# NTT123/vietTTS

Hardware: NVIDIA H100
Metric: audio_samples_per_sec (higher is better)
Workload: dtype f32 (bf16x3 split products on wgmma tensor cores, fp32 accumulate/storage)

## Files before the change

### viettts_b200/csrc/tc_conv.cu

```cuda
#include <cuda_bf16.h>

#include <algorithm>

#include "tc_common.cuh"
#include "vtts_internal.cuh"

namespace {

using namespace tcx;

constexpr int NCWG = 2;
constexpr int NCONS = NCWG * 128;
constexpr int PROD_WARP = NCONS / 32;
constexpr int NCONV = 96;
constexpr int NTHREADS = NCONS + 32 + NCONV;
constexpr int NA = 4;
constexpr int HALO = 64;
constexpr int PAIR_OVERLAP = 16;
constexpr int NQ = 2;
constexpr int NREADERS = (NCONS + NCONV) / 32;

constexpr int SUB_CG = 4;
constexpr int SUB_HALO = 1;
constexpr int SUB_RS = NCWG * 64 + SUB_HALO;
constexpr int SUB_CSB = SUB_RS * 64 + 32;
constexpr int SUB_STAGE = SUB_CG * SUB_CSB;
static_assert(SUB_RS * 4 % 32 == 4 && SUB_CSB / 4 % 32 == 24, "bank-conflict-free converter stores");

template <int N, int MW, int PAIRF, bool STAGED = false, bool SUB = false>
struct TcCfg {
  static constexpr int R = 64 * MW * NCWG;
  static constexpr int R_OUT = R - PAIR_OVERLAP;
  static constexpr int RA = R + HALO;
  static constexpr int A_STAGE = RA * 64;
  static constexpr int NAS = SUB ? (N == 64 ? 4 : 2) : NA;
  static constexpr int A_BYTES = SUB ? NAS * SUB_STAGE : NA * A_STAGE;
  static constexpr int W_STAGE = N * 64;
  static constexpr int NW = N == 256 ? 4 : 8;
  static constexpr int NCH2 = PAIRF ? N / 16 : 0;
  static constexpr int EPI_NC = N < 128 ? N : 128;
  static constexpr int EPI_LD = EPI_NC + 8;
  static constexpr int EPI_WG = 64 * EPI_LD + N;
  static constexpr int EPI_STAGE = STAGED ? NCWG * EPI_WG * 4 : 0;
  static constexpr int SMEM_BYTES =
      A_BYTES + NW * W_STAGE + NCH2 * A_STAGE + EPI_STAGE + (2 * NA + 2 * NW + 2 * NQ) * 8 + NQ * 4 + 1024;
  static_assert(SMEM_BYTES <= 227 * 1024, "shared memory of one CTA");
};

struct Ring {
  uint32_t s = 0, p = 0;
  template <int NS>
  __device__ __forceinline__ void next() { if (++s == NS) { s = 0; p ^= 1; } }
};

struct Tile {
  int pi, b, tt;
};
__device__ __forceinline__ Tile decode_tile(int t, int nprob, int tiles_per_row) {
  Tile d;
  d.pi = t % nprob; t /= nprob;
  d.tt = t % tiles_per_row;
  d.b = t / tiles_per_row;
  return d;
}

__device__ __forceinline__ int take_ticket(int* sched, int ntiles) {
  const int t = (int)gridDim.x + atomicAdd(&sched[0], 1);
  if (t < ntiles) return t;
  __threadfence();
  if (atomicAdd(&sched[1], 1) == (int)gridDim.x - 1) {
    atomicExch(&sched[0], 0);
    atomicExch(&sched[1], 0);
  }
  return -1;
}

struct TileQueue {
  int* id;
  uint64_t* full;
  uint64_t* empty;
  Ring r;
  __device__ __forceinline__ void put(int t, int* err, long long& acc) {
    mbar_wait_t(&empty[r.s], r.p ^ 1, err, 6, acc);
    id[r.s] = t;
    mbar_arrive(&full[r.s]);
    r.next<NQ>();
  }
  __device__ __forceinline__ int get(int* err, long long& acc) {
    int t = 0;
    if ((threadIdx.x & 31) == 0) {
      mbar_wait_t(&full[r.s], r.p, err, 6, acc);
      t = id[r.s];
      mbar_arrive(&empty[r.s]);
    }
    r.next<NQ>();
    return __shfl_sync(0xffffffffu, t, 0);
  }
};

__device__ __forceinline__ float div3_rn(float s) {
  constexpr float y = 0x1.555556p-2f;
  const float q0 = __fmul_rn(s, y);
  const float q1 = __fmaf_rn(__fmaf_rn(-q0, 3.0f, s), y, q0);
  return (s == 0.f || fabsf(s) == __int_as_float(0x7f800000)) ? s : q1;
}

template <int QN, int RS, int CSB, bool F16, bool LOADS_FIRST = false>
__device__ __forceinline__ void convert_rows(uint8_t* stage, int ct, const float* x0, const float* x1, const float* x2, int ld, int ch0,
                                             int row_base, int rows, int lo, int valid, int pre_mode, float slope) {
  static_assert(NCONV % QN == 0, "whole rows per converter step");
  constexpr int RSTEP = NCONV / QN, RA = RS;
  const int q = ct % QN;
  const int r0 = ct / QN;
  uint8_t* st = stage + (q >> 2) * CSB + (((q >> 1) & 1) * RA) * 16 + (q & 1) * 8;
  const int coff = ch0 + q * 4;
  constexpr int U = 8;
  for (int rr0 = r0; rr0 < rows; rr0 += RSTEP * U) {
    float4 v[U];
    if constexpr (LOADS_FIRST) {
      float4 a[U], bb[U];
      bool in[U];
#pragma unroll
      for (int u = 0; u < U; ++u) {
        const int rr = rr0 + u * RSTEP;
        const int t = row_base + rr;
        in[u] = rr < rows && t >= lo && t < valid;
        v[u] = a[u] = bb[u] = make_float4(0.f, 0.f, 0.f, 0.f);
        if (in[u]) {
          const size_t off = (size_t)t * ld + coff;
          v[u] = ldg_pf256(x0 + off);
          if (pre_mode == 2) {
            a[u] = ldg_pf256(x1 + off);
            bb[u] = ldg_pf256(x2 + off);
          }
        }
      }
#pragma unroll
      for (int u = 0; u < U; ++u) {
        if (in[u] && pre_mode == 2) {
          v[u].x = div3_rn((v[u].x + a[u].x) + bb[u].x);
          v[u].y = div3_rn((v[u].y + a[u].y) + bb[u].y);
          v[u].z = div3_rn((v[u].z + a[u].z) + bb[u].z);
          v[u].w = div3_rn((v[u].w + a[u].w) + bb[u].w);
        }
      }
    } else {
#pragma unroll
      for (int u = 0; u < U; ++u) {
        const int rr = rr0 + u * RSTEP;
        const int t = row_base + rr;
        v[u] = make_float4(0.f, 0.f, 0.f, 0.f);
        if (rr < rows && t >= lo && t < valid) {
          const size_t off = (size_t)t * ld + coff;
          v[u] = ldg_pf256(x0 + off);
          if (pre_mode == 2) {
            const float4 a = ldg_pf256(x1 + off);
            const float4 bb = ldg_pf256(x2 + off);
            v[u].x = ((v[u].x + a.x) + bb.x) / 3.0f;
            v[u].y = ((v[u].y + a.y) + bb.y) / 3.0f;
            v[u].z = ((v[u].z + a.z) + bb.z) / 3.0f;
            v[u].w = ((v[u].w + a.w) + bb.w) / 3.0f;
          }
        }
      }
    }
#pragma unroll
    for (int u = 0; u < U; ++u) {
      const int rr = rr0 + u * RSTEP;
      if (rr < rows) {
        float4 x = v[u];
        if (pre_mode >= 1) {
          x.x = lrelu(x.x, slope); x.y = lrelu(x.y, slope); x.z = lrelu(x.z, slope); x.w = lrelu(x.w, slope);
        }
        if constexpr (F16) {
          *reinterpret_cast<uint2*>(st + (size_t)rr * 16) = f16x4_sat(x);
        } else {
          uint2 hi, lo;
          split4(x, hi, lo);
          *reinterpret_cast<uint2*>(st + (size_t)rr * 16) = hi;
          *reinterpret_cast<uint2*>(st + (size_t)(2 * RA + rr) * 16) = lo;
        }
      }
    }
  }
}

template <int RA, bool F16>
__device__ __forceinline__ void convert_chunk(uint8_t* stage, int ct, const float* x0, const float* x1, const float* x2, int ld, int c,
                                              int row_base, int rows, int lo, int valid, int pre_mode, float slope) {
  convert_rows<4, RA, 0, F16>(stage, ct, x0, x1, x2, ld, c * 16, row_base, rows, lo, valid, pre_mode, slope);
}

template <int N, int NW, bool F16>
__device__ __forceinline__ void produce_weights(uint8_t* w_st, uint64_t* w_full, uint64_t* w_empty, Ring& rw, const void* wpk, int nch,
                                                int k, int* err, long long& wait_acc) {
  constexpr int WB = F16 ? N * 32 : N * 64;
  const uint8_t* src = reinterpret_cast<const uint8_t*>(wpk);
  for (int i = 0; i < nch * k; ++i) {
    mbar_wait_t(&w_empty[rw.s], rw.p ^ 1, err, 4, wait_acc);
    mbar_expect_tx(&w_full[rw.s], WB);
    bulk_g2s(w_st + rw.s * (N * 64), src + (size_t)i * WB, WB, &w_full[rw.s]);
    rw.next<NW>();
  }
}

template <int N, int MW, int RA, int NW, bool A_FROM_RING, bool A_REGS, bool F16>
__device__ __forceinline__ void consume(float (&acc)[MW][N / 2], int wg, uint32_t a_st_u32, uint64_t* a_full, uint64_t* a_empty, Ring& ra,
                                        uint32_t w_st_u32, uint64_t* w_full, uint64_t* w_empty, Ring& rw, int nch, int k, int dil,
                                        int* err, long long& w_a, long long& w_w) {
  const uint64_t a_tmpl = make_desc(0, RA * 16, 128);
  const uint64_t b_tmpl = make_desc(0, (F16 ? 1 : 2) * N * 16, 128);
  const bool lane0 = (threadIdx.x & 31) == 0;
  int pend_w = -1, pend_a = -1;
  for (int c = 0; c < nch; ++c) {
    uint32_t a_base;
    if constexpr (A_FROM_RING) {
      mbar_wait_t(&a_full[ra.s], ra.p, err, 2, w_a);
      a_base = a_st_u32 + ra.s * (RA * 64);
    } else {
      a_base = a_st_u32 + c * (RA * 64);
    }
    for (int j = 0; j < k; ++j) {
      mbar_wait_t(&w_full[rw.s], rw.p, err, 3, w_w);
      const uint32_t w_base = w_st_u32 + rw.s * (N * 64);
      const uint64_t b_hi = b_tmpl | (uint64_t)(w_base >> 4);
      const uint64_t b_lo = b_tmpl | (uint64_t)((w_base + N * 16) >> 4);
      const uint32_t first = (c | j) != 0 ? 1u : 0u;
      if constexpr (A_REGS) {
        static_assert(!A_FROM_RING && !F16, "register A operand: bf16 planes of the fixed buffer");
        const int lane = threadIdx.x & 31, wl = (threadIdx.x >> 5) & 3;
        uint32_t fa_hi[MW][4], fa_lo[MW][4];
#pragma unroll
        for (int mt = 0; mt < MW; ++mt) {
          const int row = (wg * MW + mt) * 64 + wl * 16 + ((lane >> 3) & 1) * 8 + (lane & 7) + j * dil;
          const uint32_t addr = a_base + ((lane >> 4) * RA + row) * 16;
          ldmatrix_x4(fa_hi[mt], addr);
          ldmatrix_x4(fa_lo[mt], addr + 2 * RA * 16);
        }
        wgmma_fence();
#pragma unroll
        for (int mt = 0; mt < MW; ++mt) {
          wgmma_rs<N>(acc[mt], fa_hi[mt], b_hi, first);
          wgmma_rs<N>(acc[mt], fa_hi[mt], b_lo, 1u);
          wgmma_rs<N>(acc[mt], fa_lo[mt], b_hi, 1u);
        }
        wgmma_commit();
        wgmma_wait<0>();
        if (lane == 0) mbar_arrive(&w_empty[rw.s]);
        rw.next<NW>();
        continue;
      }
      wgmma_fence();
#pragma unroll
      for (int mt = 0; mt < MW; ++mt) {
        const uint32_t row = a_base + ((wg * MW + mt) * 64 + j * dil) * 16;
        const uint64_t a_hi = a_tmpl | (uint64_t)(row >> 4);
        const uint64_t a_lo = a_tmpl | (uint64_t)((row + 2 * RA * 16) >> 4);
        if constexpr (F16) {
          wgmma<N, true>(acc[mt], a_hi, b_hi, first);
        } else {
          wgmma<N>(acc[mt], a_hi, b_hi, first);
          wgmma<N>(acc[mt], a_hi, b_lo, 1u);
          wgmma<N>(acc[mt], a_lo, b_hi, 1u);
        }
      }
      wgmma_commit();
      wgmma_wait<1>();
      if (lane0) {
        if (pend_w >= 0) mbar_arrive(&w_empty[pend_w]);
        if (pend_a >= 0) mbar_arrive(&a_empty[pend_a]);
      }
      pend_w = (int)rw.s;
      pend_a = (A_FROM_RING && j == k - 1) ? (int)ra.s : -1;
      rw.next<NW>();
    }
    if constexpr (A_FROM_RING) ra.next<NA>();
  }
  wgmma_wait<0>();
  if (lane0) {
    if (pend_w >= 0) mbar_arrive(&w_empty[pend_w]);
    if (pend_a >= 0) mbar_arrive(&a_empty[pend_a]);
  }
}

template <int N, int NW, int NAS, bool F16>
__device__ __forceinline__ void consume_rows(float (&acc)[N / 2], int wg, uint32_t a_st_u32, uint64_t* a_full, uint64_t* a_empty, Ring& ra,
                                             uint32_t w_st_u32, uint64_t* w_full, uint64_t* w_empty, Ring& rw, int nch, int k, int dil,
                                             int* err, long long& w_a, long long& w_w) {
  const uint64_t a_tmpl = make_desc(0, SUB_RS * 16, 128);
  const uint64_t b_tmpl = make_desc(0, (F16 ? 1 : 2) * N * 16, 128);
  const bool lane0 = (threadIdx.x & 31) == 0;
  int pend_w = -1, pend_a = -1;
  for (int c0 = 0; c0 < nch; c0 += SUB_CG) {
    mbar_wait_t(&a_full[ra.s], ra.p, err, 2, w_a);
    const uint32_t a_blk = a_st_u32 + ra.s * SUB_STAGE + wg * 64 * 16;
    for (int cl = 0; cl < SUB_CG; ++cl) {
      for (int j = 0; j < k; ++j) {
        mbar_wait_t(&w_full[rw.s], rw.p, err, 3, w_w);
        const uint32_t w_base = w_st_u32 + rw.s * (N * 64);
        const uint64_t b_hi = b_tmpl | (uint64_t)(w_base >> 4);
        const uint64_t b_lo = b_tmpl | (uint64_t)((w_base + N * 16) >> 4);
        const uint32_t first = ((c0 + cl) | j) != 0 ? 1u : 0u;
        const uint32_t row = a_blk + cl * SUB_CSB + j * dil * 16;
        const uint64_t a_hi = a_tmpl | (uint64_t)(row >> 4);
        const uint64_t a_lo = a_tmpl | (uint64_t)((row + 2 * SUB_RS * 16) >> 4);
        wgmma_fence();
        if constexpr (F16) {
          wgmma<N, true>(acc, a_hi, b_hi, first);
        } else {
          wgmma<N>(acc, a_hi, b_hi, first);
          wgmma<N>(acc, a_hi, b_lo, 1u);
          wgmma<N>(acc, a_lo, b_hi, 1u);
        }
        wgmma_commit();
        wgmma_wait<1>();
        if (lane0) {
          if (pend_w >= 0) mbar_arrive(&w_empty[pend_w]);
          if (pend_a >= 0) mbar_arrive(&a_empty[pend_a]);
        }
        pend_w = (int)rw.s;
        pend_a = (cl == SUB_CG - 1 && j == k - 1) ? (int)ra.s : -1;
        rw.next<NW>();
      }
    }
    ra.next<NAS>();
  }
  wgmma_wait<0>();
  if (lane0) {
    if (pend_w >= 0) mbar_arrive(&w_empty[pend_w]);
    if (pend_a >= 0) mbar_arrive(&a_empty[pend_a]);
  }
}

__device__ __forceinline__ void cp_async16(void* smem_dst, const void* gsrc) {
  asm volatile("cp.async.cg.shared.global [%0], [%1], 16;" ::"r"(smem_u32(smem_dst)), "l"(gsrc) : "memory");
}
__device__ __forceinline__ void cp_async_commit() { asm volatile("cp.async.commit_group;" ::: "memory"); }
__device__ __forceinline__ void cp_async_wait_all() { asm volatile("cp.async.wait_all;" ::: "memory"); }

__device__ __forceinline__ void init_barriers(uint64_t* bars, int nw) {
  uint64_t* a_full = bars;
  uint64_t* a_empty = bars + NA;
  uint64_t* w_full = bars + 2 * NA;
  uint64_t* w_empty = bars + 2 * NA + nw;
  uint64_t* q_full = bars + 2 * NA + 2 * nw;
  uint64_t* q_empty = q_full + NQ;
  for (int i = 0; i < NA; ++i) { mbar_init(&a_full[i], NCONV); mbar_init(&a_empty[i], NCONS / 32); }
  for (int i = 0; i < nw; ++i) { mbar_init(&w_full[i], 1); mbar_init(&w_empty[i], NCONS / 32); }
  for (int i = 0; i < NQ; ++i) { mbar_init(&q_full[i], 1); mbar_init(&q_empty[i], NREADERS); }
  asm volatile("fence.mbarrier_init.release.cluster;" ::: "memory");
}

__device__ __forceinline__ TileQueue tile_queue(uint64_t* bars, int nw) {
  uint64_t* q_full = bars + 2 * NA + 2 * nw;
  return TileQueue{reinterpret_cast<int*>(q_full + 2 * NQ), q_full, q_full + NQ, Ring{}};
}

// ... 157 lines not shown
      }
      const long long t_epi0 = clock64();
      if constexpr (EPI == 0) {
        wait_pass();
#pragma unroll
        for (int mt = 0; mt < MW; ++mt) {
          const int blk = blk_row(mt);
          if (SUB ? sub_elem(L, P, blk, 0) >= e_lim : !row_ok(blk)) break;
#pragma unroll
          for (int nh = 0; nh < N / EPI_NC; ++nh) {
            if (mt + nh > 0 && P.resid) {
              fetch_pass(mt, nh);
              wait_pass();
            }
#pragma unroll
            for (int jn = 0; jn < EPI_NC / 8; ++jn) {
              const int col = jn * 8 + fc, e = (nh * (EPI_NC / 8) + jn) * 4;
              const float2 bi = *reinterpret_cast<const float2*>(stg_bias + nh * EPI_NC + col);
#pragma unroll
              for (int h = 0; h < 2; ++h) {
                float2* s = reinterpret_cast<float2*>(stg + (fr + 8 * h) * EPI_LD + col);
                float2 o = make_float2(acc[mt][e + 2 * h] + bi.x, acc[mt][e + 2 * h + 1] + bi.y);
                if (P.resid) {
                  const float2 r = *s;
                  o.x += r.x; o.y += r.y;
                }
                *s = o;
              }
            }
            named_bar(2 + wg, 128);
#pragma unroll
            for (int i = 0; i < NQ4; ++i) {
              const int row = i * RPS + dr, tau = blk + row;
              const int e = (tau * ostride + ooff) * L.out_ld + oe0 + nh * EPI_NC + dq * 4;
              if (elem_ok(tau, e))
                *reinterpret_cast<float4*>(P.out + out_base + e) = *reinterpret_cast<const float4*>(stg + row * EPI_LD + dq * 4);
            }
            named_bar(2 + wg, 128);
          }
        }
      } else {
        const int row_w = tau0 + wg * MW * 64 + (warp & 3) * 16 + (lane >> 2);
#pragma unroll
        for (int mt = 0; mt < MW; ++mt)
#pragma unroll
          for (int h = 0; h < 2; ++h) {
            const int tau = row_w + mt * 64 + 8 * h;
            if (!row_ok(tau)) continue;
            const size_t orow = out_base + (size_t)(tau * ostride + ooff) * L.out_ld;
#pragma unroll
            for (int jn = 0; jn < N / 8; ++jn) {
              const int col = jn * 8 + 2 * (lane & 3);
              if (col >= n_valid) continue;
              float2 o = make_float2(acc[mt][jn * 4 + 2 * h], acc[mt][jn * 4 + 2 * h + 1]);
              const float2 bi = __ldg(reinterpret_cast<const float2*>(P.bias + col));
              o.x += bi.x; o.y += bi.y;
              if (P.bn_mean) {
                const float2 mu = __ldg(reinterpret_cast<const float2*>(P.bn_mean + col));
                const float2 iv = __ldg(reinterpret_cast<const float2*>(P.bn_inv + col));
                const float2 of = __ldg(reinterpret_cast<const float2*>(P.bn_off + col));
                o.x = (o.x - mu.x) * iv.x + of.x; o.y = (o.y - mu.y) * iv.y + of.y;
              }
              if (post_act == 1) { o.x = tanhf(o.x); o.y = tanhf(o.y); }
              else if (post_act == 2) { o.x = fmaxf(o.x, 0.f); o.y = fmaxf(o.y, 0.f); }
              if (P.resid) {
                const float2 r = __ldg(reinterpret_cast<const float2*>(P.resid + orow + col));
                o.x += r.x; o.y += r.y;
              }
              *reinterpret_cast<float2*>(P.out + orow + col) = o;
            }
          }
      }
      t_epi += clock64() - t_epi0;
    TILE_LOOP_END
    if (L.dbg && tid == 0) {
      long long* d = L.dbg + (size_t)blockIdx.x * 16;
      d[0] = clock64() - t_begin; d[1] = t_epi; d[2] = w_a; d[3] = w_w;
    }
  }
#undef TILE_LOOP_BEGIN
#undef TILE_LOOP_END
}

template <int N, int MW, bool A2_REGS, bool F16>
__global__ void __launch_bounds__(NTHREADS, 1) tc_pair_kernel(const __grid_constant__ TcPairLaunch L) {
  using Cfg = TcCfg<N, MW, 1>;
  constexpr int R = Cfg::R, R_OUT = Cfg::R_OUT, RA = Cfg::RA, NW = Cfg::NW, NCH = N / 16;
  extern __shared__ uint8_t smem_raw[];
  uint8_t* smem = (uint8_t*)(((uintptr_t)smem_raw + 1023) & ~(uintptr_t)1023);
  uint8_t* a_st = smem;
  uint8_t* w_st = smem + NA * Cfg::A_STAGE;
  uint8_t* mid = w_st + NW * Cfg::W_STAGE;
  uint64_t* bars = reinterpret_cast<uint64_t*>(mid + Cfg::NCH2 * Cfg::A_STAGE);
  uint64_t* a_full = bars;
  uint64_t* a_empty = bars + NA;
  uint64_t* w_full = bars + 2 * NA;
  uint64_t* w_empty = bars + 2 * NA + NW;

  const int tid = threadIdx.x;
  const int warp = __shfl_sync(0xffffffffu, tid >> 5, 0);
  if (tid == 0) init_barriers(bars, NW);
  __syncthreads();

#define TILE_LOOP_BEGIN                                                   \
  for (int tile; (tile = next_tile()) >= 0;) {                            \
    const Tile td = decode_tile(tile, L.nprob, L.tiles_per_row);        \
    const int b = td.b;                                                    \
    const int tau0 = td.tt * R_OUT;                                        \
    int valid = L.T_rows;                                                 \
    if (L.len) {                                                          \
      const int v = L.len[b] * L.len_mul;                                 \
      valid = v < valid ? v : valid;                                      \
    }                                                                     \
    if (tau0 >= valid) continue;                                          \
    const TcPairProb& P = L.p[td.pi];                                      \
    const int k = P.k, dil = P.dil, h2 = (k - 1) / 2;
#define TILE_LOOP_END }

  if (warp == PROD_WARP) {
    if ((tid & 31) == 0) {
      Ring rw;
      long long w_e = 0;
      PRODUCER_TILES
      TILE_LOOP_BEGIN
        (void)b; (void)tau0; (void)dil; (void)h2;
        produce_weights<N, NW, F16>(w_st, w_full, w_empty, rw, P.w1pk, NCH, k, L.err, w_e);
        produce_weights<N, NW, F16>(w_st, w_full, w_empty, rw, P.w2pk, NCH, k, L.err, w_e);
      TILE_LOOP_END
    }
  } else if (warp > PROD_WARP) {
    const int ct = tid - NCONS - 32;
    Ring ra;
    long long w_ae = 0;
    READER_TILES
    TILE_LOOP_BEGIN
      const float* x = P.x + (size_t)b * L.T_rows * N;
      const int row_base = tau0 - h2 - (k - 1) * dil / 2;
      for (int c = 0; c < NCH; ++c) {
        mbar_wait_t(&a_empty[ra.s], ra.p ^ 1, L.err, 5, w_ae);
        convert_chunk<RA, F16>(a_st + ra.s * Cfg::A_STAGE, ct, x, nullptr, nullptr, N, c, row_base, R + (k - 1) * dil, 0, valid, 1, L.slope);
        fence_proxy_async();
        mbar_arrive(&a_full[ra.s]);
        ra.next<NA>();
      }
    TILE_LOOP_END
  } else {
    const int wg = warp >> 2, lane = tid & 31;
    float acc[MW][N / 2];
    Ring ra, rw;
    long long w_a = 0, w_w = 0;
    const long long t_begin = clock64();
    const float slope = L.slope;
    READER_TILES
    TILE_LOOP_BEGIN
      consume<N, MW, RA, NW, true, false, F16>(acc, wg, smem_u32(a_st), a_full, a_empty, ra, smem_u32(w_st), w_full, w_empty, rw, NCH, k, dil,
                                               L.err, w_a, w_w);
      const int lr_w = wg * MW * 64 + (warp & 3) * 16 + (lane >> 2);
#pragma unroll
      for (int mt = 0; mt < MW; ++mt)
#pragma unroll
        for (int h = 0; h < 2; ++h) {
          const int lr = lr_w + mt * 64 + 8 * h;
          const int u = tau0 - h2 + lr;
          const bool inside = u >= 0 && u < valid;
#pragma unroll
          for (int jn = 0; jn < N / 8; ++jn) {
            const int col = jn * 8 + 2 * (lane & 3);
            const float2 bi = __ldg(reinterpret_cast<const float2*>(P.b1 + col));
            const float v0 = inside ? lrelu(acc[mt][jn * 4 + 2 * h] + bi.x, slope) : 0.f;
            const float v1 = inside ? lrelu(acc[mt][jn * 4 + 2 * h + 1] + bi.y, slope) : 0.f;
            uint8_t* dst = mid + (col >> 4) * Cfg::A_STAGE + (((col >> 3) & 1) * RA + lr) * 16 + (col & 7) * 2;
            if constexpr (F16) {
              *reinterpret_cast<uint32_t*>(dst) = f16x2_sat(v0, v1);
            } else {
              const __nv_bfloat162 hi = __floats2bfloat162_rn(v0, v1);
              const __nv_bfloat162 lo = __floats2bfloat162_rn(v0 - __low2float(hi), v1 - __high2float(hi));
              *reinterpret_cast<__nv_bfloat162*>(dst) = hi;
              *reinterpret_cast<__nv_bfloat162*>(dst + 2 * RA * 16) = lo;
            }
          }
        }
      fence_proxy_async();
      named_bar(1, NCONS);
      consume<N, MW, RA, NW, false, A2_REGS, F16>(acc, wg, smem_u32(mid), a_full, a_empty, ra, smem_u32(w_st), w_full, w_empty, rw, NCH, k, 1,
                                                  L.err, w_a, w_w);
      named_bar(1, NCONS);
      const float* x = P.x + (size_t)b * L.T_rows * N;
      float* out = P.out + (size_t)b * L.T_rows * N;
#pragma unroll
      for (int mt = 0; mt < MW; ++mt)
#pragma unroll
        for (int h = 0; h < 2; ++h) {
          const int lr = lr_w + mt * 64 + 8 * h;
          const int tau = tau0 + lr;
          if (lr >= R_OUT || tau >= valid) continue;
#pragma unroll
          for (int jn = 0; jn < N / 8; ++jn) {
            const int col = jn * 8 + 2 * (lane & 3);
            const float2 bi = __ldg(reinterpret_cast<const float2*>(P.b2 + col));
            const float2 r = __ldg(reinterpret_cast<const float2*>(x + (size_t)tau * N + col));
            float2 o;
            o.x = acc[mt][jn * 4 + 2 * h] + bi.x + r.x;
            o.y = acc[mt][jn * 4 + 2 * h + 1] + bi.y + r.y;
            *reinterpret_cast<float2*>(out + (size_t)tau * N + col) = o;
          }
        }
    TILE_LOOP_END
    if (L.dbg && tid == 0) {
      long long* d = L.dbg + (size_t)blockIdx.x * 16;
      d[0] = clock64() - t_begin; d[2] = w_a; d[3] = w_w;
    }
  }
#undef TILE_LOOP_BEGIN
#undef TILE_LOOP_END
}

template <bool F16>
__global__ void pack_w_kernel(const float* __restrict__ w, uint16_t* __restrict__ dst, int k, int Cin, int Cout_total, int n0, int N) {
  const size_t total = (size_t)k * Cin * N;
  for (size_t idx = blockIdx.x * (size_t)blockDim.x + threadIdx.x; idx < total; idx += (size_t)gridDim.x * blockDim.x) {
    const int n = idx % N;
    const int i = (idx / N) % Cin;
    const int j = idx / ((size_t)N * Cin);
    const float v = (n0 + n) < Cout_total ? w[((size_t)j * Cin + i) * Cout_total + n0 + n] : 0.f;
    const int c = i / 16, kh = (i % 16) / 8, e = i % 8;
    if constexpr (F16) {
      const size_t blk = ((size_t)c * k + j) * (size_t)(2 * N * 8);
      dst[blk + ((size_t)kh * N + n) * 8 + e] = (uint16_t)(f16x2_sat(v, 0.f) & 0xffffu);
      continue;
    }
    const __nv_bfloat16 hi = __float2bfloat16_rn(v);
    const __nv_bfloat16 lo = __float2bfloat16_rn(v - __bfloat162float(hi));
    const size_t blk = ((size_t)c * k + j) * (size_t)(4 * N * 8);
    dst[blk + ((size_t)(kh * 2 + 0) * N + n) * 8 + e] = __bfloat16_as_ushort(hi);
    dst[blk + ((size_t)(kh * 2 + 1) * N + n) * 8 + e] = __bfloat16_as_ushort(lo);
  }
}

template <int N, int EPI, int MW, bool F16, bool SUB = false>
int launch_cfg(vtts_ctx* ctx, TcLaunch& L, cudaStream_t st) {
  using Cfg = TcCfg<N, MW, 0, EPI == 0, SUB>;
  static bool attr_done_dev[64] = {};
  if (!attr_done_dev[ctx->device & 63]) {
    VTTS_CUDA(cudaFuncSetAttribute(tc_conv_kernel<N, EPI, MW, F16, SUB>, cudaFuncAttributeMaxDynamicSharedMemorySize, Cfg::SMEM_BYTES));
    attr_done_dev[ctx->device & 63] = true;
  }
  for (int i = 0; i < L.nprob; ++i)
    if ((L.p[i].k - 1) * L.p[i].dil > (SUB ? SUB_HALO : HALO)) return ctx->fail(VTTS_ERR_BAD_ARG, "tc_conv: halo too large");
  if (SUB && L.Cin % (SUB_CG * 16)) return ctx->fail(VTTS_ERR_BAD_ARG, "tc_conv: sub-row output needs Cin %% %d == 0, not %d", SUB_CG * 16, L.Cin);
  std::stable_sort(L.p, L.p + L.nprob, [](const TcProb& a, const TcProb& b) { return a.k > b.k; });
  L.tiles_per_row = ((L.tile_rows > 0 ? L.tile_rows : L.T_rows) + Cfg::R - 1) / Cfg::R;
  L.ntiles = L.nprob * L.tiles_per_row * L.B;
  const int grid = L.ntiles < ctx->sm_count ? L.ntiles : ctx->sm_count;
  tc_conv_kernel<N, EPI, MW, F16, SUB><<<grid, NTHREADS, Cfg::SMEM_BYTES, st>>>(L);
  ctx->launches++;
  VTTS_CUDA(cudaGetLastError());
  return VTTS_OK;
}

template <int N>
int launch_n(vtts_ctx* ctx, TcLaunch& L, cudaStream_t st) {
  constexpr int MW = N >= 256 ? 1 : (N == 128 ? 2 : 4);
  bool generic = L.post_act != 0 || (L.n_valid > 0 && L.n_valid < N);
  bool rb = false;
  for (int i = 0; i < L.nprob; ++i) {
    generic |= L.p[i].bn_mean != nullptr;
    rb |= L.p[i].rb != nullptr;
  }
  if ((rb || L.out_sub) && generic) return ctx->fail(VTTS_ERR_BAD_ARG, "tc_conv: per-row bounds and sub-row output use the plain epilogue");
  if (L.out_sub < 0 || (L.out_sub && (L.out_sub % 4 || L.out_ld % L.out_sub)))
    return ctx->fail(VTTS_ERR_BAD_ARG, "tc_conv: output rows of %d floats in tile rows of %d", L.out_sub, L.out_ld);
  if (!generic) {
    const int row_w = L.out_sub ? L.out_sub : L.out_ld;
    if ((int64_t)L.rows_out * row_w > INT32_MAX) return ctx->fail(VTTS_ERR_BAD_ARG, "tc_conv: %d output rows of %d", L.rows_out, row_w);
    bool aligned = L.out_ld % 4 == 0;
    for (int i = 0; i < L.nprob; ++i) aligned &= (((uintptr_t)L.p[i].out | (uintptr_t)L.p[i].resid | (uintptr_t)L.p[i].bias) & 15) == 0;
    if (!aligned) return ctx->fail(VTTS_ERR_BAD_ARG, "tc_conv: the plain epilogue needs 16-byte aligned out / resid rows and bias (out_ld %d)", L.out_ld);
  }
  if (L.f16 && generic) return ctx->fail(VTTS_ERR_BAD_ARG, "tc_conv: fp16 operands use the plain epilogue");
  if (L.f16) return L.out_sub ? launch_cfg<N, 0, MW, true, true>(ctx, L, st) : launch_cfg<N, 0, MW, true>(ctx, L, st);
  if (generic) return launch_cfg<N, 1, MW, false>(ctx, L, st);
  return L.out_sub ? launch_cfg<N, 0, MW, false, true>(ctx, L, st) : launch_cfg<N, 0, MW, false>(ctx, L, st);
}

template <int N, int MW, bool A2_REGS, bool F16 = false>
int launch_pair(vtts_ctx* ctx, TcPairLaunch& L, cudaStream_t st) {
  using Cfg = TcCfg<N, MW, 1>;
  static bool attr_done_dev[64] = {};
  if (!attr_done_dev[ctx->device & 63]) {
    VTTS_CUDA(cudaFuncSetAttribute(tc_pair_kernel<N, MW, A2_REGS, F16>, cudaFuncAttributeMaxDynamicSharedMemorySize, Cfg::SMEM_BYTES));
    attr_done_dev[ctx->device & 63] = true;
  }
  for (int i = 0; i < L.nprob; ++i)
    if (L.p[i].k - 1 > PAIR_OVERLAP || (L.p[i].k - 1) * L.p[i].dil > HALO) return ctx->fail(VTTS_ERR_BAD_ARG, "tc_pair: halo too large");
  std::stable_sort(L.p, L.p + L.nprob, [](const TcPairProb& a, const TcPairProb& b) { return a.k > b.k; });
  L.tiles_per_row = (L.T_rows + Cfg::R_OUT - 1) / Cfg::R_OUT;
  L.ntiles = L.nprob * L.tiles_per_row * L.B;
  const int grid = L.ntiles < ctx->sm_count ? L.ntiles : ctx->sm_count;
  tc_pair_kernel<N, MW, A2_REGS, F16><<<grid, NTHREADS, Cfg::SMEM_BYTES, st>>>(L);
  ctx->launches++;
  VTTS_CUDA(cudaGetLastError());
  return VTTS_OK;
}

}

size_t vtts_tc_packed_elems(int k, int Cin, int N, bool f16) { return (size_t)k * Cin * N * (f16 ? 1 : 2); }

int vtts_tc_pack_weights(vtts_ctx* ctx, const float* w, void* dst, int k, int Cin, int Cout_total, int n0, int N, bool f16) {
  if (f16) pack_w_kernel<true><<<256, 256>>>(w, reinterpret_cast<uint16_t*>(dst), k, Cin, Cout_total, n0, N);
  else pack_w_kernel<false><<<256, 256>>>(w, reinterpret_cast<uint16_t*>(dst), k, Cin, Cout_total, n0, N);
  VTTS_CUDA(cudaGetLastError());
  return VTTS_OK;
}

int vtts_tc_tile_n(int Cout) { return Cout <= 32 ? 32 : (Cout <= 64 ? 64 : (Cout <= 128 ? 128 : 256)); }

size_t vtts_tc_conv_packed_bytes(int k, int Cin, int Cout, bool f16) {
  const int N = vtts_tc_tile_n(Cout), nt = (Cout + N - 1) / N;
  return ((vtts_tc_packed_elems(k, Cin, N, f16) * 2 + 255) & ~size_t(255)) * nt;
}

int vtts_tc_pack_conv(vtts_ctx* ctx, const float* w, int k, int Cin, int Cout, bool f16, char*& cursor, std::vector<void*>& out) {
  const int N = vtts_tc_tile_n(Cout), nt = (Cout + N - 1) / N;
  for (int t = 0; t < nt; ++t) {
    int rc = vtts_tc_pack_weights(ctx, w, cursor, k, Cin, Cout, t * N, N, f16);
    if (rc) return rc;
    out.push_back(cursor);
    cursor += (vtts_tc_packed_elems(k, Cin, N, f16) * 2 + 255) & ~size_t(255);
  }
  return VTTS_OK;
}

int vtts_conv_dispatch(vtts_ctx* ctx, const ConvLaunch& L, void* const* wpk, cudaStream_t st) {
  if (ctx->precision == VTTS_PRECISION_FP32 || wpk == nullptr) return vtts_launch_conv(ctx, L, st);
  const int N = vtts_tc_tile_n(L.Cout), nt = (L.Cout + N - 1) / N;
  TcLaunch TL;
  auto reset = [&]() {
    memset(&TL, 0, sizeof(TL));
    TL.Cin = L.Cin; TL.N = N; TL.in_ld = L.Cin; TL.out_ld = L.Cout; TL.B = L.B; TL.T_rows = L.T_rows; TL.rows_out = L.rows_out;
    TL.len = L.len; TL.len_mul = L.len_mul; TL.pre_mode = L.pre_mode; TL.pre_slope = L.pre_slope; TL.post_act = L.post_act;
    TL.n_valid = (L.Cout % N) ? (L.Cout % N) : N;
  };
  reset();
  for (int pass = 0; pass < 2; ++pass) {
    const bool partial = pass == 1;
    if (partial && (L.Cout % N) == 0) break;
    reset();
    TL.n_valid = partial ? (L.Cout % N) : N;
    for (int pi = 0; pi < L.nprob; ++pi) {
      const ConvProb& cp = L.p[pi];
      for (int t = 0; t < nt; ++t) {
        const bool is_partial = (t == nt - 1) && (L.Cout % N) != 0;
        if (is_partial != partial) continue;
        const int n0 = t * N;
        TcProb q;
        memset(&q, 0, sizeof(q));
        q.x0 = cp.x0; q.x1 = cp.x1; q.x2 = cp.x2;
        q.wpk = wpk[pi * nt + t];
        q.bias = cp.bias + n0;
        q.resid = cp.resid ? cp.resid + n0 : nullptr;
        if (cp.bn_mean) { q.bn_mean = cp.bn_mean + n0; q.bn_inv = cp.bn_inv + n0; q.bn_off = cp.bn_off + n0; }
        q.out = cp.out + n0;
        q.k = cp.k; q.dil = cp.dil; q.in_off = cp.in_off; q.out_stride = cp.out_stride; q.out_off = cp.out_off;
        TL.p[TL.nprob++] = q;
        if (TL.nprob == 8) {
          int rc = vtts_launch_tc_conv(ctx, TL, st);
          if (rc) return rc;
          TL.nprob = 0;
        }
      }
    }
    if (TL.nprob > 0) {
      int rc = vtts_launch_tc_conv(ctx, TL, st);
      if (rc) return rc;
    }
  }
  return VTTS_OK;
}

int vtts_launch_tc_conv(vtts_ctx* ctx, TcLaunch& L, cudaStream_t st) {
  if (L.nprob < 1 || L.nprob > 8) return ctx->fail(VTTS_ERR_BAD_ARG, "tc_conv: nprob %d", L.nprob);
  if (L.Cin % 16 != 0) return ctx->fail(VTTS_ERR_BAD_ARG, "tc_conv: Cin %d", L.Cin);
  for (int i = 0; i < L.nprob; ++i)
    if (L.p[i].k < 1) return ctx->fail(VTTS_ERR_BAD_ARG, "tc_conv: k");
  L.sched = ctx->d_tc_sched;
  L.err = ctx->d_err;
  L.dbg = ctx->tc_dbg_on ? ctx->d_tc_dbg : nullptr;
  switch (L.N) {
    case 256: return launch_n<256>(ctx, L, st);
    case 128: return launch_n<128>(ctx, L, st);
    case 64: return launch_n<64>(ctx, L, st);
    case 32: return launch_n<32>(ctx, L, st);
    default: return ctx->fail(VTTS_ERR_BAD_ARG, "tc_conv: N %d unsupported", L.N);
  }
}

int vtts_launch_tc_pair(vtts_ctx* ctx, TcPairLaunch& L, cudaStream_t st) {
  if (L.nprob < 1 || L.nprob > 3) return ctx->fail(VTTS_ERR_BAD_ARG, "tc_pair: nprob %d", L.nprob);
  for (int i = 0; i < L.nprob; ++i)
    if (L.p[i].k < 1 || L.p[i].x == L.p[i].out) return ctx->fail(VTTS_ERR_BAD_ARG, "tc_pair: bad problem %d", i);
  L.sched = ctx->d_tc_sched;
  L.err = ctx->d_err;
  L.dbg = ctx->tc_dbg_on ? ctx->d_tc_dbg : nullptr;
  if (L.N != 32 && L.N != 64) return ctx->fail(VTTS_ERR_BAD_ARG, "tc_pair: C %d unsupported (32 or 64)", L.N);
  if (L.f16) {
    if (ctx->pair_ts != 2) return ctx->fail(VTTS_ERR_BAD_ARG, "tc_pair: fp16 operands exist for the default pair form (256-row tiles) only, not form %d", ctx->pair_ts);
    return L.N == 64 ? launch_pair<64, 2, false, true>(ctx, L, st) : launch_pair<32, 2, false, true>(ctx, L, st);
  }
  if (ctx->pair_ts == 1) return L.N == 64 ? launch_pair<64, 2, true>(ctx, L, st) : launch_pair<32, 2, true>(ctx, L, st);
  if (ctx->pair_ts == 0) return L.N == 64 ? launch_pair<64, 1, false>(ctx, L, st) : launch_pair<32, 1, false>(ctx, L, st);
  return L.N == 64 ? launch_pair<64, 2, false>(ctx, L, st) : launch_pair<32, 2, false>(ctx, L, st);
}
```

### viettts_b200/csrc/vtts_internal.cuh

```cuda
#pragma once
#include <cuda_runtime.h>
#include <stdint.h>
#include <stdio.h>
#include <string.h>
#include <algorithm>
#include <string>
#include <vector>

#include "../../include/viettts_b200.h"

namespace vc {
constexpr int MEL = 80;
constexpr int HOP = 256;
constexpr int NFFT = 1024;
constexpr int NBINS = 513;
constexpr int ENC_D = 256;
constexpr int ENC_OUT = 512;
constexpr int DEC_H = 512;
constexpr int PRENET = 256;
constexpr int POSTNET = 512;
constexpr int VOCAB = 256;
constexpr int SIL_INDEX = 0;
constexpr int WORD_END_INDEX = 3;
constexpr int LAUNCH_ROWS = 128;
// ... 20 lines not shown
  const float* x2;
  const float* w;
  const float* bias;
  const float* resid;
  const float* bn_mean;
  const float* bn_inv;
  const float* bn_off;
  float* out;
  int k, dil, in_off;
  int out_stride, out_off;
};

struct ConvLaunch {
  ConvProb p[8];
  int nprob;
  int Cin, Cout;
  int B;
  int T_rows;
  int rows_out;
  const int* len;
  int len_mul;
  int pre_mode;
  float pre_slope;
  int post_act;
};

struct TcProb {
  const float* x0;
  const float* x1;
  const float* x2;
  const void* wpk;
  const float* bias;
  const float* resid;
  const float* bn_mean;
  const float* bn_inv;
  const float* bn_off;
  float* out;
  int k, dil, in_off, out_stride, out_off;
  int out_e0;
  const int* rb;
};

struct TcLaunch {
  TcProb p[8];
  int nprob;
  int Cin, N;
  int in_ld, out_ld;
  int B, T_rows, rows_out;
  const int* len;
  int len_mul;
  int pre_mode;
  float pre_slope;
  int out_sub;
  int post_act;
  int n_valid;
  int f16;
  int tile_rows;
  int tiles_per_row, ntiles;
  int* sched;
  int* err;
  long long* dbg;
};

struct TcPairProb {
  const float* x;
  const void* w1pk;
  const void* w2pk;
  const float* b1;
  const float* b2;
  float* out;
  int k, dil;
};

struct TcPairLaunch {
  TcPairProb p[3];
  int nprob;
  int N;
  int B, T_rows;
  const int* len;
  int len_mul;
  float slope;
  int f16;
  int tiles_per_row, ntiles;
  int* sched;
  int* err;
  long long* dbg;
};

struct ModelWeights {
  float* blob = nullptr;
  std::vector<float*> t;
  float* derived = nullptr;
  std::vector<float*> d;
  void* wpk = nullptr;
  std::vector<void*> wpk_t;
  std::vector<int> tile0;
  bool loaded = false;
  void* const* tiles(int conv) const { return &wpk_t[tile0[conv]]; }
};

struct vtts_ctx {
  int device = 0;
  int precision = 1;
  int* d_err = nullptr;
  int* d_tc_sched = nullptr;
  long long* d_tc_dbg = nullptr;
  bool tc_dbg_on = false;
  int fuse_pairs = 1;
  int pair_ts = 2;
  int sm_count = 0;
  int cc_major = 0, cc_minor = 0;
  size_t hbm_bytes = 0;
  std::string err;
  int64_t launches = 0;
  cudaStream_t own_stream = nullptr;

  ModelWeights hg;
  ModelWeights ac;
  ModelWeights du;

  float* mel_fb = nullptr;
  int* mel_lo = nullptr;
  int* mel_hi = nullptr;
  float* fft_tw = nullptr;
  float* hann = nullptr;
  bool fft_ready = false;
  bool mel_loaded = false;

  void* ws = nullptr;
  size_t ws_bytes = 0;
  void* hpin = nullptr;
  size_t hpin_bytes = 0;
  void* dstage = nullptr;
  size_t dstage_bytes = 0;

  struct RsFilter { int up, down; float* taps; };
  std::vector<RsFilter> rs_filters;
  struct LnFilter { int rate; float coef[10]; float seg[5][16]; float blk[16]; };
  std::vector<LnFilter> ln_filters;

  float* tap_enc = nullptr; int64_t tap_enc_n = 0;
  float* tap_cond = nullptr; int64_t tap_cond_n = 0;
  float* tap_melpre = nullptr; int64_t tap_melpre_n = 0;
  float* tap_decin = nullptr; int64_t tap_decin_n = 0;
  float* tap_decout = nullptr; int64_t tap_decout_n = 0;
  float* tap_durhid = nullptr; int64_t tap_durhid_n = 0;
  void clear_taps() {
    tap_enc = tap_cond = tap_melpre = tap_decin = tap_decout = tap_durhid = nullptr;
    tap_enc_n = tap_cond_n = tap_melpre_n = tap_decin_n = tap_decout_n = tap_durhid_n = 0;
  }

  static constexpr int NSTAGE = 4;
  cudaEvent_t ev0[NSTAGE] = {nullptr, nullptr, nullptr, nullptr};
  cudaEvent_t ev1[NSTAGE] = {nullptr, nullptr, nullptr, nullptr};
  cudaStream_t ev_stream[NSTAGE] = {nullptr, nullptr, nullptr, nullptr};
  bool ev_valid[NSTAGE] = {false, false, false, false};

  static constexpr int NSUB = 24;
  bool sub_on = false;
  cudaEvent_t sub_ev[NSUB] = {};
  bool sub_set[NSUB] = {};
  void sub_mark(int id, cudaStream_t st) {
    if (!sub_on) return;
    if (!sub_ev[id]) cudaEventCreate(&sub_ev[id]);
    cudaEventRecord(sub_ev[id], st);
    sub_set[id] = true;
// ... 178 lines not shown
```

Baseline: 57.66 million.

## Keep pair-conv weights resident in shared memory for C=32 with banded tile scheduling

For C=32 pair convolutions with k<=11, the producer loads both convs' full weight sets into shared memory once per problem switch instead of streaming per-chunk weight stages for every tile. Tiles are reordered in bands so each CTA processes tiles of the same problem consecutively, and consumers skip per-step weight barrier waits. The change also prefetches the residual and bias before the second GEMM and doubles the converter unroll. This cuts redundant weight traffic and barrier overhead, at the cost of much larger shared memory, more registers, and a new schedule decoding path.

```diff
diff --git a/viettts_b200/csrc/tc_conv.cu b/viettts_b200/csrc/tc_conv.cu
--- a/viettts_b200/csrc/tc_conv.cu
+++ b/viettts_b200/csrc/tc_conv.cu
@@ -105,7 +105,7 @@
   return (s == 0.f || fabsf(s) == __int_as_float(0x7f800000)) ? s : q1;
 }
 
-template <int QN, int RS, int CSB, bool F16, bool LOADS_FIRST = false>
+template <int QN, int RS, int CSB, bool F16, bool LOADS_FIRST = false, int U = 8>
 __device__ __forceinline__ void convert_rows(uint8_t* stage, int ct, const float* x0, const float* x1, const float* x2, int ld, int ch0,
                                              int row_base, int rows, int lo, int valid, int pre_mode, float slope) {
   static_assert(NCONV % QN == 0, "whole rows per converter step");
@@ -114,7 +114,6 @@
   const int r0 = ct / QN;
   uint8_t* st = stage + (q >> 2) * CSB + (((q >> 1) & 1) * RA) * 16 + (q & 1) * 8;
   const int coff = ch0 + q * 4;
-  constexpr int U = 8;
   for (int rr0 = r0; rr0 < rows; rr0 += RSTEP * U) {
     float4 v[U];
     if constexpr (LOADS_FIRST) {
@@ -185,10 +184,10 @@
   }
 }
 
-template <int RA, bool F16>
+template <int RA, bool F16, int U = 8>
 __device__ __forceinline__ void convert_chunk(uint8_t* stage, int ct, const float* x0, const float* x1, const float* x2, int ld, int c,
                                               int row_base, int rows, int lo, int valid, int pre_mode, float slope) {
-  convert_rows<4, RA, 0, F16>(stage, ct, x0, x1, x2, ld, c * 16, row_base, rows, lo, valid, pre_mode, slope);
+  convert_rows<4, RA, 0, F16, false, U>(stage, ct, x0, x1, x2, ld, c * 16, row_base, rows, lo, valid, pre_mode, slope);
 }
 
 template <int N, int NW, bool F16>
@@ -204,7 +203,7 @@
   }
 }
 
-template <int N, int MW, int RA, int NW, bool A_FROM_RING, bool A_REGS, bool F16>
+template <int N, int MW, int RA, int NW, bool A_FROM_RING, bool A_REGS, bool F16, bool W_RES = false>
 __device__ __forceinline__ void consume(float (&acc)[MW][N / 2], int wg, uint32_t a_st_u32, uint64_t* a_full, uint64_t* a_empty, Ring& ra,
                                         uint32_t w_st_u32, uint64_t* w_full, uint64_t* w_empty, Ring& rw, int nch, int k, int dil,
                                         int* err, long long& w_a, long long& w_w) {
@@ -221,12 +220,18 @@
       a_base = a_st_u32 + c * (RA * 64);
     }
     for (int j = 0; j < k; ++j) {
-      mbar_wait_t(&w_full[rw.s], rw.p, err, 3, w_w);
-      const uint32_t w_base = w_st_u32 + rw.s * (N * 64);
+      uint32_t w_base;
+      if constexpr (W_RES) {
+        w_base = w_st_u32 + (c * k + j) * (F16 ? N * 32 : N * 64);
+      } else {
+        mbar_wait_t(&w_full[rw.s], rw.p, err, 3, w_w);
+        w_base = w_st_u32 + rw.s * (N * 64);
+      }
       const uint64_t b_hi = b_tmpl | (uint64_t)(w_base >> 4);
       const uint64_t b_lo = b_tmpl | (uint64_t)((w_base + N * 16) >> 4);
       const uint32_t first = (c | j) != 0 ? 1u : 0u;
       if constexpr (A_REGS) {
+        static_assert(!W_RES, "register A operand: streamed weights");
         static_assert(!A_FROM_RING && !F16, "register A operand: bf16 planes of the fixed buffer");
         const int lane = threadIdx.x & 31, wl = (threadIdx.x >> 5) & 3;
         uint32_t fa_hi[MW][4], fa_lo[MW][4];
@@ -270,9 +275,11 @@
         if (pend_w >= 0) mbar_arrive(&w_empty[pend_w]);
         if (pend_a >= 0) mbar_arrive(&a_empty[pend_a]);
       }
-      pend_w = (int)rw.s;
       pend_a = (A_FROM_RING && j == k - 1) ? (int)ra.s : -1;
-      rw.next<NW>();
+      if constexpr (!W_RES) {
+        pend_w = (int)rw.s;
+        rw.next<NW>();
+      }
     }
     if constexpr (A_FROM_RING) ra.next<NA>();
   }
@@ -596,15 +603,54 @@
 #undef TILE_LOOP_END
 }
 
-template <int N, int MW, bool A2_REGS, bool F16>
+constexpr int PAIR_RES_KMAX = 11;
+template <int N, bool F16>
+struct PairRes {
+  using Cfg = TcCfg<N, 2, 1>;
+  static constexpr int WB = F16 ? N * 32 : N * 64;
+  static constexpr int FIXED = NA * Cfg::A_STAGE + Cfg::NCH2 * Cfg::A_STAGE + (2 * NA + 2 + 2 * NQ) * 8 + NQ * 4 + 1024;
+  static constexpr int W_BYTES_MAX = 2 * (N / 16) * PAIR_RES_KMAX * WB;
+  static constexpr int SMEM_MAX = FIXED + W_BYTES_MAX;
+  static int smem_bytes(int kmax) { return FIXED + 2 * (N / 16) * kmax * WB; }
+};
+
+struct PairTile {
+  int pi, b, tau0, valid;
+};
+__device__ __forceinline__ Tile decode_pair_tile(const TcPairLaunch& L, int t) {
+  if (L.band == 0) return decode_tile(t, L.nprob, L.tiles_per_row);
+  const int per = L.band * L.nprob, band = t / per, g0 = band * L.band;
+  const int s = min(L.band, L.B * L.tiles_per_row - g0);
+  const int r = t - band * per, g = g0 + r % s;
+  Tile d;
+  d.pi = r / s;
+  d.b = g / L.tiles_per_row;
+  d.tt = g % L.tiles_per_row;
+  return d;
+}
+__device__ __forceinline__ bool pair_tile(const TcPairLaunch& L, int t, int r_out, PairTile& d) {
+  const Tile td = decode_pair_tile(L, t);
+  d.pi = td.pi; d.b = td.b; d.tau0 = td.tt * r_out;
+  d.valid = L.T_rows;
+  if (L.len) {
+    const int v = L.len[td.b] * L.len_mul;
+    d.valid = v < d.valid ? v : d.valid;
+  }
+  return d.tau0 < d.valid;
+}
+
+template <int N, int MW, bool A2_REGS, bool F16, bool RES>
 __global__ void __launch_bounds__(NTHREADS, 1) tc_pair_kernel(const __grid_constant__ TcPairLaunch L) {
+  static_assert(!RES || (N == 32 && MW == 2 && !A2_REGS), "resident weights: C = 32, 256-row tiles, A operands in shared memory");
+  static_assert(!RES || PairRes<N, F16>::SMEM_MAX <= 227 * 1024, "shared memory of one CTA with resident pair weights");
   using Cfg = TcCfg<N, MW, 1>;
-  constexpr int R = Cfg::R, R_OUT = Cfg::R_OUT, RA = Cfg::RA, NW = Cfg::NW, NCH = N / 16;
+  constexpr int R = Cfg::R, R_OUT = Cfg::R_OUT, RA = Cfg::RA, NW = RES ? 1 : Cfg::NW, NCH = N / 16;
+  constexpr int WB = PairRes<N, F16>::WB;
   extern __shared__ uint8_t smem_raw[];
   uint8_t* smem = (uint8_t*)(((uintptr_t)smem_raw + 1023) & ~(uintptr_t)1023);
   uint8_t* a_st = smem;
   uint8_t* w_st = smem + NA * Cfg::A_STAGE;
-  uint8_t* mid = w_st + NW * Cfg::W_STAGE;
+  uint8_t* mid = w_st + (RES ? 2 * NCH * L.p[0].k * WB : NW * Cfg::W_STAGE);
   uint64_t* bars = reinterpret_cast<uint64_t*>(mid + Cfg::NCH2 * Cfg::A_STAGE);
   uint64_t* a_full = bars;
   uint64_t* a_empty = bars + NA;
@@ -618,15 +664,9 @@
 
 #define TILE_LOOP_BEGIN                                                   \
   for (int tile; (tile = next_tile()) >= 0;) {                            \
-    const Tile td = decode_tile(tile, L.nprob, L.tiles_per_row);        \
-    const int b = td.b;                                                    \
-    const int tau0 = td.tt * R_OUT;                                        \
-    int valid = L.T_rows;                                                 \
-    if (L.len) {                                                          \
-      const int v = L.len[b] * L.len_mul;                                 \
-      valid = v < valid ? v : valid;                                      \
-    }                                                                     \
-    if (tau0 >= valid) continue;                                          \
+    PairTile td;                                                          \
+    if (!pair_tile(L, tile, R_OUT, td)) continue;                         \
+    const int b = td.b, tau0 = td.tau0, valid = td.valid;                 \
     const TcPairProb& P = L.p[td.pi];                                      \
     const int k = P.k, dil = P.dil, h2 = (k - 1) / 2;
 #define TILE_LOOP_END }
@@ -634,13 +674,31 @@
   if (warp == PROD_WARP) {
     if ((tid & 31) == 0) {
       Ring rw;
-      long long w_e = 0;
+      long long w_e = 0, loads = 0;
+      int w_pi = -1;
       PRODUCER_TILES
       TILE_LOOP_BEGIN
-        (void)b; (void)tau0; (void)dil; (void)h2;
-        produce_weights<N, NW, F16>(w_st, w_full, w_empty, rw, P.w1pk, NCH, k, L.err, w_e);
-        produce_weights<N, NW, F16>(w_st, w_full, w_empty, rw, P.w2pk, NCH, k, L.err, w_e);
+        (void)b; (void)tau0; (void)valid; (void)dil; (void)h2;
+        if constexpr (RES) {
+          if (td.pi != w_pi) {
+            if (loads > 0) mbar_wait_t(w_empty, (uint32_t)(loads - 1) & 1, L.err, 4, w_e);
+            const uint32_t bytes = NCH * k * WB;
+            mbar_expect_tx(w_full, 2 * bytes);
+            bulk_g2s(w_st, P.w1pk, bytes, w_full);
+            bulk_g2s(w_st + bytes, P.w2pk, bytes, w_full);
+            w_pi = td.pi;
+            ++loads;
+          }
+        } else {
+          produce_weights<N, NW, F16>(w_st, w_full, w_empty, rw, P.w1pk, NCH, k, L.err, w_e);
+          produce_weights<N, NW, F16>(w_st, w_full, w_empty, rw, P.w2pk, NCH, k, L.err, w_e);
+          ++loads;
+        }
       TILE_LOOP_END
+      if (L.dbg) {
+        L.dbg[(size_t)blockIdx.x * 16 + 4] = w_e;
+        L.dbg[(size_t)blockIdx.x * 16 + 10] = loads;
+      }
     }
   } else if (warp > PROD_WARP) {
     const int ct = tid - NCONS - 32;
@@ -652,23 +710,45 @@
       const int row_base = tau0 - h2 - (k - 1) * dil / 2;
       for (int c = 0; c < NCH; ++c) {
         mbar_wait_t(&a_empty[ra.s], ra.p ^ 1, L.err, 5, w_ae);
-        convert_chunk<RA, F16>(a_st + ra.s * Cfg::A_STAGE, ct, x, nullptr, nullptr, N, c, row_base, R + (k - 1) * dil, 0, valid, 1, L.slope);
+        convert_chunk<RA, F16, RES ? 16 : 8>(a_st + ra.s * Cfg::A_STAGE, ct, x, nullptr, nullptr, N, c, row_base, R + (k - 1) * dil, 0, valid,
+                                              1, L.slope);
         fence_proxy_async();
         mbar_arrive(&a_full[ra.s]);
         ra.next<NA>();
       }
     TILE_LOOP_END
+    if (L.dbg && ct == 0) L.dbg[(size_t)blockIdx.x * 16 + 5] = w_ae;
   } else {
     const int wg = warp >> 2, lane = tid & 31;
     float acc[MW][N / 2];
     Ring ra, rw;
-    long long w_a = 0, w_w = 0;
+    long long w_a = 0, w_w = 0, t_mid = 0, t_epi = 0;
     const long long t_begin = clock64();
     const float slope = L.slope;
+    const uint32_t w1_u32 = smem_u32(w_st);
     READER_TILES
-    TILE_LOOP_BEGIN
-      consume<N, MW, RA, NW, true, false, F16>(acc, wg, smem_u32(a_st), a_full, a_empty, ra, smem_u32(w_st), w_full, w_empty, rw, NCH, k, dil,
-                                               L.err, w_a, w_w);
+    auto next_live = [&]() {
+      PairTile d;
+      for (int t; (t = next_tile()) >= 0;)
+        if (pair_tile(L, t, R_OUT, d)) return d;
+      d.pi = -1;
+      return d;
+    };
+    int w_pi = -1;
+    uint32_t w_ph = 0;
+    for (PairTile td = next_live(); td.pi >= 0;) {
+      const int b = td.b, tau0 = td.tau0, valid = td.valid;
+      const TcPairProb& P = L.p[td.pi];
+      const int k = P.k, dil = P.dil, h2 = (k - 1) / 2;
+      if (RES && td.pi != w_pi) {
+        mbar_wait_t(w_full, w_ph, L.err, 3, w_w);
+        w_ph ^= 1;
+        w_pi = td.pi;
+      }
+      const uint32_t w2_u32 = w1_u32 + (RES ? NCH * k * WB : 0);
+      consume<N, MW, RA, NW, true, false, F16, RES>(acc, wg, smem_u32(a_st), a_full, a_empty, ra, w1_u32, w_full, w_empty, rw, NCH, k, dil,
+                                                    L.err, w_a, w_w);
+      const long long t_mid0 = clock64();
       const int lr_w = wg * MW * 64 + (warp & 3) * 16 + (lane >> 2);
 #pragma unroll
       for (int mt = 0; mt < MW; ++mt)
@@ -696,10 +776,34 @@
         }
       fence_proxy_async();
       named_bar(1, NCONS);
-      consume<N, MW, RA, NW, false, A2_REGS, F16>(acc, wg, smem_u32(mid), a_full, a_empty, ra, smem_u32(w_st), w_full, w_empty, rw, NCH, k, 1,
-                                                  L.err, w_a, w_w);
+      t_mid += clock64() - t_mid0;
+      const float* x = P.x + (size_t)b * L.T_rows * N;
+      float2 pre_r[RES ? MW : 1][2][N / 8], pre_b2[N / 8];
+      if constexpr (RES) {
+#pragma unroll
+        for (int jn = 0; jn < N / 8; ++jn) pre_b2[jn] = __ldg(reinterpret_cast<const float2*>(P.b2 + jn * 8 + 2 * (lane & 3)));
+#pragma unroll
+        for (int mt = 0; mt < MW; ++mt)
+#pragma unroll
+          for (int h = 0; h < 2; ++h) {
+            const int lr = lr_w + mt * 64 + 8 * h;
+            const int tau = tau0 + lr;
+            const bool ok = lr < R_OUT && tau < valid;
+#pragma unroll
+            for (int jn = 0; jn < N / 8; ++jn)
+              pre_r[mt][h][jn] = ok ? __ldg(reinterpret_cast<const float2*>(x + (size_t)tau * N + jn * 8 + 2 * (lane & 3)))
+                                    : make_float2(0.f, 0.f);
+          }
+      }
+      consume<N, MW, RA, NW, false, A2_REGS, F16, RES>(acc, wg, smem_u32(mid), a_full, a_empty, ra, w2_u32, w_full, w_empty, rw, NCH, k, 1,
+                                                       L.err, w_a, w_w);
       named_bar(1, NCONS);
-      const float* x = P.x + (size_t)b * L.T_rows * N;
+      PairTile nx;
+      if constexpr (RES) {
+        nx = next_live();
+        if (nx.pi >= 0 && nx.pi != td.pi && lane == 0) mbar_arrive(w_empty);
+      }
+      const long long t_epi0 = clock64();
       float* out = P.out + (size_t)b * L.T_rows * N;
 #pragma unroll
       for (int mt = 0; mt < MW; ++mt)
@@ -711,18 +815,21 @@
 #pragma unroll
           for (int jn = 0; jn < N / 8; ++jn) {
             const int col = jn * 8 + 2 * (lane & 3);
-            const float2 bi = __ldg(reinterpret_cast<const float2*>(P.b2 + col));
-            const float2 r = __ldg(reinterpret_cast<const float2*>(x + (size_t)tau * N + col));
+            const float2 bi = RES ? pre_b2[jn] : __ldg(reinterpret_cast<const float2*>(P.b2 + col));
+            const float2 r = RES ? pre_r[RES ? mt : 0][h][jn] : __ldg(reinterpret_cast<const float2*>(x + (size_t)tau * N + col));
             float2 o;
             o.x = acc[mt][jn * 4 + 2 * h] + bi.x + r.x;
             o.y = acc[mt][jn * 4 + 2 * h + 1] + bi.y + r.y;
             *reinterpret_cast<float2*>(out + (size_t)tau * N + col) = o;
           }
         }
-    TILE_LOOP_END
+      t_epi += clock64() - t_epi0;
+      if constexpr (!RES) nx = next_live();
+      td = nx;
+    }
     if (L.dbg && tid == 0) {
       long long* d = L.dbg + (size_t)blockIdx.x * 16;
-      d[0] = clock64() - t_begin; d[2] = w_a; d[3] = w_w;
+      d[0] = clock64() - t_begin; d[1] = t_epi; d[2] = w_a; d[3] = w_w; d[9] = t_mid;
     }
   }
 #undef TILE_LOOP_BEGIN
@@ -797,21 +904,27 @@
   return L.out_sub ? launch_cfg<N, 0, MW, false, true>(ctx, L, st) : launch_cfg<N, 0, MW, false>(ctx, L, st);
 }
 
-template <int N, int MW, bool A2_REGS, bool F16 = false>
+constexpr int PAIR_BAND_PER_CTA = 3;
+
+template <int N, int MW, bool A2_REGS, bool F16 = false, bool RES = false>
 int launch_pair(vtts_ctx* ctx, TcPairLaunch& L, cudaStream_t st) {
   using Cfg = TcCfg<N, MW, 1>;
   static bool attr_done_dev[64] = {};
   if (!attr_done_dev[ctx->device & 63]) {
-    VTTS_CUDA(cudaFuncSetAttribute(tc_pair_kernel<N, MW, A2_REGS, F16>, cudaFuncAttributeMaxDynamicSharedMemorySize, Cfg::SMEM_BYTES));
+    VTTS_CUDA(cudaFuncSetAttribute(tc_pair_kernel<N, MW, A2_REGS, F16, RES>, cudaFuncAttributeMaxDynamicSharedMemorySize,
+                                   RES ? PairRes<N, F16>::SMEM_MAX : Cfg::SMEM_BYTES));
     attr_done_dev[ctx->device & 63] = true;
   }
   for (int i = 0; i < L.nprob; ++i)
     if (L.p[i].k - 1 > PAIR_OVERLAP || (L.p[i].k - 1) * L.p[i].dil > HALO) return ctx->fail(VTTS_ERR_BAD_ARG, "tc_pair: halo too large");
   std::stable_sort(L.p, L.p + L.nprob, [](const TcPairProb& a, const TcPairProb& b) { return a.k > b.k; });
+  if (RES && L.p[0].k > PAIR_RES_KMAX) return ctx->fail(VTTS_ERR_BAD_ARG, "tc_pair: resident weights need k <= %d", PAIR_RES_KMAX);
   L.tiles_per_row = (L.T_rows + Cfg::R_OUT - 1) / Cfg::R_OUT;
   L.ntiles = L.nprob * L.tiles_per_row * L.B;
   const int grid = L.ntiles < ctx->sm_count ? L.ntiles : ctx->sm_count;
-  tc_pair_kernel<N, MW, A2_REGS, F16><<<grid, NTHREADS, Cfg::SMEM_BYTES, st>>>(L);
+  L.band = RES ? PAIR_BAND_PER_CTA * grid : 0;
+  const int smem = RES ? PairRes<N, F16>::smem_bytes(L.p[0].k) : Cfg::SMEM_BYTES;
+  tc_pair_kernel<N, MW, A2_REGS, F16, RES><<<grid, NTHREADS, smem, st>>>(L);
   ctx->launches++;
   VTTS_CUDA(cudaGetLastError());
   return VTTS_OK;
@@ -918,11 +1031,16 @@
   L.err = ctx->d_err;
   L.dbg = ctx->tc_dbg_on ? ctx->d_tc_dbg : nullptr;
   if (L.N != 32 && L.N != 64) return ctx->fail(VTTS_ERR_BAD_ARG, "tc_pair: C %d unsupported (32 or 64)", L.N);
+  int kmax = 0;
+  for (int i = 0; i < L.nprob; ++i) kmax = std::max(kmax, L.p[i].k);
+  const bool res = L.N == 32 && kmax <= PAIR_RES_KMAX;
   if (L.f16) {
     if (ctx->pair_ts != 2) return ctx->fail(VTTS_ERR_BAD_ARG, "tc_pair: fp16 operands exist for the default pair form (256-row tiles) only, not form %d", ctx->pair_ts);
-    return L.N == 64 ? launch_pair<64, 2, false, true>(ctx, L, st) : launch_pair<32, 2, false, true>(ctx, L, st);
+    if (L.N == 64) return launch_pair<64, 2, false, true>(ctx, L, st);
+    return res ? launch_pair<32, 2, false, true, true>(ctx, L, st) : launch_pair<32, 2, false, true>(ctx, L, st);
   }
   if (ctx->pair_ts == 1) return L.N == 64 ? launch_pair<64, 2, true>(ctx, L, st) : launch_pair<32, 2, true>(ctx, L, st);
   if (ctx->pair_ts == 0) return L.N == 64 ? launch_pair<64, 1, false>(ctx, L, st) : launch_pair<32, 1, false>(ctx, L, st);
-  return L.N == 64 ? launch_pair<64, 2, false>(ctx, L, st) : launch_pair<32, 2, false>(ctx, L, st);
-}
+  if (L.N == 64) return launch_pair<64, 2, false>(ctx, L, st);
+  return res ? launch_pair<32, 2, false, false, true>(ctx, L, st) : launch_pair<32, 2, false>(ctx, L, st);
+}
diff --git a/viettts_b200/csrc/vtts_internal.cuh b/viettts_b200/csrc/vtts_internal.cuh
--- a/viettts_b200/csrc/vtts_internal.cuh
+++ b/viettts_b200/csrc/vtts_internal.cuh
@@ -126,6 +126,7 @@
   float slope;
   int f16;
   int tiles_per_row, ntiles;
+  int band;
   int* sched;
   int* err;
   long long* dbg;
```

Result: no change. 58.15 million, median of 6 (+0.9%).
